# actcwlf/GSVC

Hardware: NVIDIA B200
Metric: train_iters_per_s (higher is better)
Workload: dtype f32

## Files before the change

gsvc_b200/csrc/common.cuh:

```cuda
#pragma once

#include <cuda_runtime.h>
#include <stdint.h>
#include <stddef.h>

#include "../../include/gsvc_rast.h"

namespace gsvc {

constexpr int TILE = GSVC_RAST_TILE;
constexpr int TILE_PIX = TILE * TILE;
constexpr float ALPHA_MIN = 1.0f / 255.0f;
constexpr float ALPHA_MAX = 0.99f;
constexpr float T_STOP = 0.0001f;
constexpr float LOWPASS = 0.3f;

constexpr int MAX_VIEWS = GSVC_RAST_MAX_VIEWS;
struct ViewTable {
    const float* V[MAX_VIEWS];
    long long vs_r[MAX_VIEWS], vs_c[MAX_VIEWS];
    float campos[MAX_VIEWS][3];
    int out_image[MAX_VIEWS];
    int flip_x[MAX_VIEWS];
    float weight[MAX_VIEWS];
};

struct DevSettings {
    int W, H, gx, gy;
    float x_min, y_min, scale, threshold, scale_modifier;
    const float* bg;
    int sh_degree, sh_M;
    int n_views, accumulate;
    ViewTable vt;
};

struct GeomView {
    float4* feat0;
    float4* feat1;
    float4* feat2;
    float4* feat3;
    ushort4* rect;
    uint8_t* clamped;
};

struct ImageHeader {
    unsigned long long num_rendered;
    unsigned int overflow;
    unsigned int n_heavy;
    unsigned int pad[28];
};
struct ImageView {
    ImageHeader* hdr;
    unsigned int* tile_count;
    unsigned long long* scan_partials;
    unsigned int* tile_offset;
    unsigned int* tile_cursor;
    uint2* ranges;
    unsigned int* heavy_tiles;
    float* final_T;
    unsigned int* n_contrib;
};

struct BinView {
    unsigned long long* inst;
    unsigned int* point_list;
    unsigned int* depth_keys;
};

__host__ __device__ inline size_t align_up(size_t x, size_t a) { return (x + a - 1) / a * a; }

template <typename T>
__host__ __device__ inline T* carve(char*& p, size_t count)
{
    T* r = reinterpret_cast<T*>(p);
    p += align_up(count * sizeof(T), 256);
    return r;
}

inline GeomView geom_view(void* buf, int P, int sh_M)
{
    char* p = static_cast<char*>(buf);
    GeomView g;
    g.feat0 = carve<float4>(p, P);
    g.feat1 = carve<float4>(p, P);
    g.feat2 = carve<float4>(p, P);
    g.feat3 = carve<float4>(p, P);
    g.rect = carve<ushort4>(p, P);
    g.clamped = sh_M > 0 ? carve<uint8_t>(p, (size_t)P * 3) : nullptr;
    return g;
}
inline size_t geom_bytes(int P, int sh_M)
{
    char* p = nullptr;
    carve<float4>(p, P); carve<float4>(p, P); carve<float4>(p, P); carve<float4>(p, P); carve<ushort4>(p, P);
    if (sh_M > 0) carve<uint8_t>(p, (size_t)P * 3);
    return (size_t)p + 256;
}
inline ImageView image_view(void* buf, int W, int H, int n_views = 1)
{
    char* p = static_cast<char*>(buf);
    size_t T = (size_t)((W + TILE - 1) / TILE) * ((H + TILE - 1) / TILE) * n_views;
    size_t N = (size_t)W * H * n_views;
    ImageView v;
    v.hdr = carve<ImageHeader>(p, 1);
    v.tile_count = carve<unsigned int>(p, T);
    v.scan_partials = carve<unsigned long long>(p, T / 1024 + 2);
    v.tile_offset = carve<unsigned int>(p, T);
    v.tile_cursor = carve<unsigned int>(p, T);
    v.ranges = carve<uint2>(p, T);
    v.heavy_tiles = carve<unsigned int>(p, T);
    v.final_T = carve<float>(p, N);
    v.n_contrib = carve<unsigned int>(p, N);
    return v;
}
inline size_t image_bytes(int W, int H, int n_views = 1)
{
    char* p = nullptr;
    size_t T = (size_t)((W + TILE - 1) / TILE) * ((H + TILE - 1) / TILE) * n_views;
    size_t N = (size_t)W * H * n_views;
    carve<ImageHeader>(p, 1); carve<unsigned int>(p, T); carve<unsigned long long>(p, T / 1024 + 2);
    carve<unsigned int>(p, T); carve<unsigned int>(p, T); carve<uint2>(p, T); carve<unsigned int>(p, T); carve<float>(p, N);
    carve<unsigned int>(p, N);
    return (size_t)p + 256;
}
inline BinView bin_view(void* buf, long long cap)
{
    char* p = static_cast<char*>(buf);
    BinView b;
    b.inst = carve<unsigned long long>(p, (size_t)cap);
    b.point_list = carve<unsigned int>(p, (size_t)cap);
    b.depth_keys = carve<unsigned int>(p, (size_t)cap);
    return b;
}
inline size_t bin_bytes(long long cap)
{
    char* p = nullptr;
    carve<unsigned long long>(p, (size_t)cap); carve<unsigned int>(p, (size_t)cap); carve<unsigned int>(p, (size_t)cap);
    return (size_t)p + 256;
}

inline size_t bwd_scratch_bytes(int P) { return align_up((size_t)P * 48, 256) + 256; }

__host__ __device__ inline unsigned int ordered_u32(float z)
{
#ifdef __CUDA_ARCH__
    unsigned int u = __float_as_uint(z);
#else
    unsigned int u; memcpy(&u, &z, 4);
#endif
    return (u & 0x80000000u) ? ~u : (u | 0x80000000u);
}

__device__ __forceinline__ float4 ld_row4(const float* __restrict__ base, size_t row)
{
    if ((reinterpret_cast<uintptr_t>(base) & 15u) == 0u) return __ldg(reinterpret_cast<const float4*>(base) + row);
    const float* p = base + 4 * row;
    return make_float4(__ldg(p), __ldg(p + 1), __ldg(p + 2), __ldg(p + 3));
}
__device__ __forceinline__ void st_row4(float* __restrict__ base, size_t row, float4 v)
{
    if ((reinterpret_cast<uintptr_t>(base) & 15u) == 0u) { reinterpret_cast<float4*>(base)[row] = v; return; }
    float* p = base + 4 * row;
    p[0] = v.x; p[1] = v.y; p[2] = v.z; p[3] = v.w;
}

#define GSVC_MUL(a, b) __fmul_rn((a), (b))
#define GSVC_ADD(a, b) __fadd_rn((a), (b))
#define GSVC_SUB(a, b) __fsub_rn((a), (b))

__device__ __forceinline__ void quat_to_rot(const float4 q, float R[9])
{
    const float r = q.x, x = q.y, y = q.z, z = q.w;
    R[0] = GSVC_SUB(1.f, GSVC_MUL(2.f, GSVC_ADD(GSVC_MUL(y, y), GSVC_MUL(z, z))));
    R[1] = GSVC_MUL(2.f, GSVC_SUB(GSVC_MUL(x, y), GSVC_MUL(r, z)));
    R[2] = GSVC_MUL(2.f, GSVC_ADD(GSVC_MUL(x, z), GSVC_MUL(r, y)));
    R[3] = GSVC_MUL(2.f, GSVC_ADD(GSVC_MUL(x, y), GSVC_MUL(r, z)));
    R[4] = GSVC_SUB(1.f, GSVC_MUL(2.f, GSVC_ADD(GSVC_MUL(x, x), GSVC_MUL(z, z))));
    R[5] = GSVC_MUL(2.f, GSVC_SUB(GSVC_MUL(y, z), GSVC_MUL(r, x)));
    R[6] = GSVC_MUL(2.f, GSVC_SUB(GSVC_MUL(x, z), GSVC_MUL(r, y)));
    R[7] = GSVC_MUL(2.f, GSVC_ADD(GSVC_MUL(y, z), GSVC_MUL(r, x)));
    R[8] = GSVC_SUB(1.f, GSVC_MUL(2.f, GSVC_ADD(GSVC_MUL(x, x), GSVC_MUL(y, y))));
}

__device__ __forceinline__ float dot3_rn(float a0, float b0, float a1, float b1, float a2, float b2)
{
    return GSVC_ADD(GSVC_ADD(GSVC_MUL(a0, b0), GSVC_MUL(a1, b1)), GSVC_MUL(a2, b2));
}

__device__ __forceinline__ void cov3d_from_scale_rot(const float* s3, float mod, const float4 q, float cov[6])
{
    float R[9], M[9];
    quat_to_rot(q, R);
    const float sx = GSVC_MUL(mod, s3[0]), sy = GSVC_MUL(mod, s3[1]), sz = GSVC_MUL(mod, s3[2]);
#pragma unroll
    for (int i = 0; i < 3; i++) {
        M[3 * i + 0] = GSVC_MUL(R[3 * i + 0], sx);
        M[3 * i + 1] = GSVC_MUL(R[3 * i + 1], sy);
        M[3 * i + 2] = GSVC_MUL(R[3 * i + 2], sz);
    }
    cov[0] = dot3_rn(M[0], M[0], M[1], M[1], M[2], M[2]);
    cov[1] = dot3_rn(M[0], M[3], M[1], M[4], M[2], M[5]);
    cov[2] = dot3_rn(M[0], M[6], M[1], M[7], M[2], M[8]);
    cov[3] = dot3_rn(M[3], M[3], M[4], M[4], M[5], M[5]);
    cov[4] = dot3_rn(M[3], M[6], M[4], M[7], M[5], M[8]);
    cov[5] = dot3_rn(M[6], M[6], M[7], M[7], M[8], M[8]);
}

__device__ __forceinline__ void cov2d_ortho(const float cov[6], const float w0[3], const float w1[3], float scale,
                                            float& a, float& b, float& c)
{
    const float u00 = dot3_rn(cov[0], w0[0], cov[1], w0[1], cov[2], w0[2]);
    const float u01 = dot3_rn(cov[1], w0[0], cov[3], w0[1], cov[4], w0[2]);
    const float u02 = dot3_rn(cov[2], w0[0], cov[4], w0[1], cov[5], w0[2]);
    const float u10 = dot3_rn(cov[0], w1[0], cov[1], w1[1], cov[2], w1[2]);
    const float u11 = dot3_rn(cov[1], w1[0], cov[3], w1[1], cov[4], w1[2]);
    const float u12 = dot3_rn(cov[2], w1[0], cov[4], w1[1], cov[5], w1[2]);
    const float s2 = GSVC_MUL(scale, scale);
    a = GSVC_ADD(GSVC_MUL(s2, dot3_rn(w0[0], u00, w0[1], u01, w0[2], u02)), LOWPASS);
    b = GSVC_MUL(s2, dot3_rn(w0[0], u10, w0[1], u11, w0[2], u12));
    c = GSVC_ADD(GSVC_MUL(s2, dot3_rn(w1[0], u10, w1[1], u11, w1[2], u12)), LOWPASS);
}

__device__ __forceinline__ void pdl_prologue()
{
#if defined(__CUDA_ARCH__)
    asm volatile("griddepcontrol.launch_dependents;");
    asm volatile("griddepcontrol.wait;" ::: "memory");
#endif
}

template <typename... KArgs, typename... Args>
inline cudaError_t launch_pdl(void (*kernel)(KArgs...), dim3 grid, dim3 block, cudaStream_t st, Args... args)
{
    cudaLaunchConfig_t cfg = {};
    cfg.gridDim = grid;
    cfg.blockDim = block;
    cfg.dynamicSmemBytes = 0;
    cfg.stream = st;
    cudaLaunchAttribute attr[1];
    attr[0].id = cudaLaunchAttributeProgrammaticStreamSerialization;
    attr[0].val.programmaticStreamSerializationAllowed = 1;
    cfg.attrs = attr;
    cfg.numAttrs = 1;
    return cudaLaunchKernelEx(&cfg, kernel, KArgs(args)...);
}

struct WarpTiles {
    int incl, excl, total;
    int rx, ry, rw;
};

__device__ __forceinline__ WarpTiles warp_tiles_begin(int area, int rx, int ry, int rw)
{
    const int lane = threadIdx.x & 31;
    int v = area;
#pragma unroll
    for (int d = 1; d < 32; d <<= 1) {
        const int o = __shfl_up_sync(0xffffffffu, v, d);
        if (lane >= d) v += o;
    }
    WarpTiles w;
    w.incl = v; w.excl = v - area; w.total = __shfl_sync(0xffffffffu, v, 31);
    w.rx = rx; w.ry = ry; w.rw = rw;
    return w;
}

__device__ __forceinline__ int warp_tiles_get(const WarpTiles& w, int idx, int gx, int& owner)
{
    int o = 0;
#pragma unroll
    for (int step = 16; step >= 1; step >>= 1) {
        const int v = __shfl_sync(0xffffffffu, w.incl, o + step - 1);
        if (v <= idx) o += step;
    }
    o = min(o, 31);
    const int local = idx - __shfl_sync(0xffffffffu, w.excl, o);
    const int rw = __shfl_sync(0xffffffffu, w.rw, o);
    const int rx = __shfl_sync(0xffffffffu, w.rx, o), ry = __shfl_sync(0xffffffffu, w.ry, o);
    owner = o;
    if (idx >= w.total) return -1;
    int row = __float2int_rz(__fdividef(__int2float_rz(local), __int2float_rz(rw)));
    int rem = local - row * rw;
    if (rem < 0) { row--; rem += rw; }
    else if (rem >= rw) { row++; rem -= rw; }
    return (ry + row) * gx + rx + rem;
}

struct PreInputs {
    int P;
    const float* means3D;
    const float* shs;
    const float* colors_precomp;
    const float* opacities;
    const float* scales;
    const float* rotations;
    const float* cov3D_precomp;
    int range_lo, range_hi;
};

cudaError_t launch_visible_filter(const DevSettings& s, const PreInputs& in, int32_t* radii, cudaStream_t st);
inline size_t compact_scratch_bytes(int P)
{
    const size_t n = ((size_t)(P < 1 ? 1 : P) + 255) / 256;
    return 256 + 2 * align_up(n * 4, 256) + align_up(n * 32, 256) + 256;
}
cudaError_t launch_visible_filter_compact(const DevSettings& s, const PreInputs& in, int32_t* radii, int32_t* indices,
                                          void* scratch, unsigned long long* host_slot, unsigned int ticket,
                                          cudaStream_t st);
cudaError_t launch_preprocess(const DevSettings& s, const PreInputs& in, int32_t* radii, GeomView g, ImageView im,
                              float4* acc_to_zero, cudaStream_t st);
cudaError_t launch_tile_scan(const DevSettings& s, ImageView im, unsigned long long* host_slot, unsigned int ticket,
                             cudaStream_t st);
cudaError_t launch_scatter(const DevSettings& s, int P, GeomView g, ImageView im, BinView b, long long cap,
                           bool count_overflow_events, cudaStream_t st);
cudaError_t launch_sort_tiles(const DevSettings& s, ImageView im, BinView b, long long cap, cudaStream_t st);
cudaError_t launch_render_forward(const DevSettings& s, GeomView g, ImageView im, BinView b, long long cap,
                                  float* out_color, cudaStream_t st);
cudaError_t launch_render_backward(const DevSettings& s, int P, GeomView g, ImageView im, BinView b, long long cap,
                                   const float* dL_dout, float4* acc, bool acc_is_zero, cudaStream_t st);
struct BwdOutputs {
    float* dL_dmeans3D; float* dL_dmeans2D; float* dL_dcolors; float* dL_dopacities;
    float* dL_dscales; float* dL_drotations; float* dL_dcov3D; float* dL_dshs;
    float* packed;
};
struct ExchangeArgs {
    float4* mc;
    float4* const* bufs;
    unsigned int* const* pads;
    unsigned int* state;
    int rank, world;
    int n_ex;
    int chunk_ctas, n_chunks;
    int n_compute;
    long long chunk_f4, total_f4;
};
cudaError_t launch_preprocess_backward(const DevSettings& s, const PreInputs& in, const int32_t* radii, GeomView g,
                                       const float4* acc, BwdOutputs out, ExchangeArgs ex, cudaStream_t st);
cudaError_t launch_export_keys(const DevSettings& s, ImageView im, BinView b, long long R,
                               unsigned long long* sorted_keys, unsigned int* point_list, unsigned int* ranges,
                               cudaStream_t st);
cudaError_t launch_export_geom(int P, GeomView g, float* depth, float* xy, float* conic_opacity, float* rgb,
                               int32_t* rect, cudaStream_t st);

cudaError_t read_overflow_events(unsigned int* host_value, bool reset, cudaStream_t st);
cudaError_t launch_densify_stats(int n_views, int P, const float* dm2d, const int32_t* radii, float* stats,
                                 long long stride, bool accumulate, cudaStream_t st);

cudaError_t launch_switch_allreduce(float* multicast, void* const* buffers, unsigned int* const* pads, unsigned int* state,
                                    int rank, int world, long long numel, int n_ctas, cudaStream_t st);
void count_launch(int n = 1);

}
```

gsvc_b200/csrc/render.cu:

```cuda
#include "common.cuh"

namespace gsvc {

constexpr int BLEND_THREADS = 128;
constexpr int BATCH = 256;
constexpr unsigned FULL = 0xffffffffu;

__device__ __forceinline__ float ex2_approx(float x)
{
    float y;
    asm("ex2.approx.ftz.f32 %0, %1;" : "=f"(y) : "f"(x));
    return y;
}
__device__ __forceinline__ float rcp_approx(float x)
{
    float y;
    asm("rcp.approx.ftz.f32 %0, %1;" : "=f"(y) : "f"(x));
    return y;
}

struct f2 { unsigned long long v; };
__device__ __forceinline__ f2 mk2(float lo, float hi)
{
    f2 r;
    asm("mov.b64 %0, {%1, %2};" : "=l"(r.v) : "f"(lo), "f"(hi));
    return r;
}
__device__ __forceinline__ f2 bc2(float s) { return mk2(s, s); }
__device__ __forceinline__ float lo(f2 a)
{
    float x;
    [[maybe_unused]] float y;
    asm("mov.b64 {%0, %1}, %2;" : "=f"(x), "=f"(y) : "l"(a.v));
    return x;
}
__device__ __forceinline__ float hi(f2 a)
{
    [[maybe_unused]] float x;
    float y;
    asm("mov.b64 {%0, %1}, %2;" : "=f"(x), "=f"(y) : "l"(a.v));
    return y;
}
__device__ __forceinline__ f2 fma2(f2 a, f2 b, f2 c)
{
    f2 r;
    asm("fma.rn.f32x2 %0, %1, %2, %3;" : "=l"(r.v) : "l"(a.v), "l"(b.v), "l"(c.v));
    return r;
}
__device__ __forceinline__ void fma2_acc(f2& c, f2 a, f2 b)
{
    asm("fma.rn.f32x2 %0, %1, %2, %0;" : "+l"(c.v) : "l"(a.v), "l"(b.v));
}
__device__ __forceinline__ f2 mul2(f2 a, f2 b)
{
    f2 r;
    asm("mul.rn.f32x2 %0, %1, %2;" : "=l"(r.v) : "l"(a.v), "l"(b.v));
    return r;
}
__device__ __forceinline__ f2 add2(f2 a, f2 b)
{
    f2 r;
    asm("add.rn.f32x2 %0, %1, %2;" : "=l"(r.v) : "l"(a.v), "l"(b.v));
    return r;
}
__device__ __forceinline__ f2 sub2(f2 a, f2 b)
{
    f2 r;
    asm("sub.rn.f32x2 %0, %1, %2;" : "=l"(r.v) : "l"(a.v), "l"(b.v));
    return r;
}
__device__ __forceinline__ f2 neg2(f2 a) { return mk2(-lo(a), -hi(a)); }

__device__ __forceinline__ f2 neg_falloff_log2(float rho_hi, const float4 f1, float dx, f2 dy2, f2& u2, f2& v2)
{
    const f2 t2 = fma2(bc2(f1.y), dy2, fma2(bc2(rho_hi), dy2, bc2(dx)));
    u2 = mul2(bc2(f1.x), t2);
    v2 = mul2(bc2(f1.z), dy2);
    return fma2(u2, u2, mul2(v2, v2));
}
__device__ __forceinline__ f2 neg_falloff_log2(float rho_hi, const float4 f1, float dx, f2 dy2)
{
    f2 u2, v2;
    return neg_falloff_log2(rho_hi, f1, dx, dy2, u2, v2);
}

struct BlockGeom {
    int px, py;
    float xmin, xmax, ymin, ymax;
};

__device__ __forceinline__ BlockGeom block_geom(int tile, int gx, int tid)
{
    const int tx = tile % gx, ty = tile / gx;
    const int warp = tid >> 5, lane = tid & 31;
    const int bx0 = tx * TILE + (warp & 1) * 8, by0 = ty * TILE + (warp >> 1) * 8;
    BlockGeom b;
    b.px = bx0 + (lane & 7);
    b.py = by0 + (lane >> 3);
    b.xmin = (float)bx0; b.xmax = (float)(bx0 + 7);
    b.ymin = (float)by0; b.ymax = (float)(by0 + 7);
    return b;
}

constexpr float CULL_MARGIN = 1e-3f;

__device__ __forceinline__ void stage(float4* s_feat, int slot, const GeomView& geo, unsigned int id)
{
    const float4 f0 = __ldg(geo.feat0 + id);
    const float4 f1 = __ldg(geo.feat3 + id);
    float4 f2 = __ldg(geo.feat2 + id);
    f2.w = __uint_as_float(id);
    s_feat[3 * slot] = f0;
    s_feat[3 * slot + 1] = f1;
    s_feat[3 * slot + 2] = f2;
}

__device__ __forceinline__ bool block_hit(const BlockGeom& b, const float4* e)
{
    const float4 f0 = e[0];
    const float4 f1 = e[1];
    const float thr = -__log2f(255.0f * f1.w) - CULL_MARGIN;
    const float ex = fminf(fmaxf(f0.x, b.xmin), b.xmax), ey = fminf(fmaxf(f0.y, b.ymin), b.ymax);
    const float dxe = ex - f0.x, dye = ey - f0.y;
    const float dy1 = fminf(fmaxf(fmaf(-f0.w, dxe, f0.y), b.ymin), b.ymax) - f0.y;
    const float dx2 = fminf(fmaxf(fmaf(-f0.z, dye, f0.x), b.xmin), b.xmax) - f0.x;
    const float u1 = f1.x * fmaf(f0.z, dy1, dxe), v1 = f1.z * dy1;
    const float u2 = f1.x * fmaf(f0.z, dye, dx2), v2 = f1.z * dye;
    const float nq1 = fmaf(u1, u1, v1 * v1), nq2 = fmaf(u2, u2, v2 * v2);
    return -fminf(nq1, nq2) >= thr;
}

__global__ void __launch_bounds__(BLEND_THREADS)
render_forward_kernel(DevSettings s, GeomView geo, ImageView im, BinView bin, unsigned long long cap,
                      float* __restrict__ out_color)
{
    __shared__ float4 s_feat[3 * BATCH];

    pdl_prologue();
    const int Tv = s.gx * s.gy;
    const int view = (int)blockIdx.x / Tv;
    const int tile = (int)blockIdx.x - view * Tv;
    const int tid = threadIdx.x, lane = tid & 31;
    const BlockGeom bg = block_geom(tile, s.gx, tid);
    const bool inA = bg.px < s.W && bg.py < s.H, inB = bg.px < s.W && bg.py + 4 < s.H;
    const float pxf = (float)bg.px, pyf = (float)bg.py;

    const uint2 rg = im.ranges[blockIdx.x];
    if ((unsigned long long)rg.y > cap) return;
    const int n = (int)(rg.y - rg.x);

    float TA = 1.f, A0 = 0.f, A1 = 0.f, A2 = 0.f;
    float TB = 1.f, B0 = 0.f, B1 = 0.f, B2 = 0.f;
    const f2 npy2 = mk2(-pyf, -(pyf + 4.f));
    unsigned int lastA = 0, lastB = 0;
    constexpr float DONE = 2.f;
    float minA = inA ? ALPHA_MIN : DONE, minB = inB ? ALPHA_MIN : DONE;

    for (int base = 0; base < n; base += BATCH) {
        if (__syncthreads_count(minA > 1.f && minB > 1.f) == BLEND_THREADS) break;
#pragma unroll
        for (int r = 0; r < BATCH / BLEND_THREADS; r++) {
            const int slot = tid + r * BLEND_THREADS;
            if (base + slot < n) stage(s_feat, slot, geo, bin.point_list[rg.x + base + slot]);
        }
        __syncthreads();
        const int cnt = min(BATCH, n - base);
        for (int c = 0; c < cnt; c += 32) {
            if (__ballot_sync(FULL, !(minA > 1.f && minB > 1.f)) == 0u) break;
            bool hit = false;
            if (c + lane < cnt) hit = block_hit(bg, s_feat + 3 * (c + lane));
            unsigned int m = __ballot_sync(FULL, hit);
            const float4* chunk = s_feat + 3 * c;
            const unsigned int pos1 = (unsigned int)(base + c + 1);
            while (m) {
                const int k = __ffs(m) - 1;
                m &= m - 1;
                const float4* e = chunk + 3 * k;
                const float4 f0 = e[0];
                const float4 f1 = e[1];
                const float4 f2v = e[2];
                const f2 nq2 = neg_falloff_log2(f0.z, f1, f0.x - pxf, add2(bc2(f0.y), npy2));
                const f2 a2 = mul2(bc2(f1.w), mk2(ex2_approx(-lo(nq2)), ex2_approx(-hi(nq2))));
                const float aA = fminf(ALPHA_MAX, lo(a2)), aB = fminf(ALPHA_MAX, hi(a2));
                const bool okA = !(aA < minA);
                const bool okB = !(aB < minB);
                const unsigned int pos = pos1 + (unsigned int)k;
                const f2 ac = mk2(aA, aB), T2 = mk2(TA, TB);
                const f2 tT2 = mul2(T2, sub2(bc2(1.f), ac));
                const f2 w2 = mul2(ac, T2);
                const float tTA = lo(tT2), tTB = hi(tT2);
                if (okA && tTA < T_STOP) minA = DONE;
                if (okB && tTB < T_STOP) minB = DONE;
                const bool addA = okA && !(tTA < T_STOP), addB = okB && !(tTB < T_STOP);
                const f2 wz = mk2(addA ? lo(w2) : 0.f, addB ? hi(w2) : 0.f);
                { const f2 c = fma2(bc2(f2v.x), wz, mk2(A0, B0)); A0 = lo(c); B0 = hi(c); }
                { const f2 c = fma2(bc2(f2v.y), wz, mk2(A1, B1)); A1 = lo(c); B1 = hi(c); }
                { const f2 c = fma2(bc2(f2v.z), wz, mk2(A2, B2)); A2 = lo(c); B2 = hi(c); }
                if (addA) { TA = tTA; lastA = pos; }
                if (addB) { TB = tTB; lastB = pos; }
            }
        }
    }
    const size_t N = (size_t)s.W * s.H;
    const float bg0 = __ldg(s.bg + 0), bg1 = __ldg(s.bg + 1), bg2 = __ldg(s.bg + 2);
    float* const fT = im.final_T + (size_t)view * N;
    unsigned int* const nc = im.n_contrib + (size_t)view * N;
    float* const out = out_color + (size_t)s.vt.out_image[view] * 3 * N;
    const float wgt = s.vt.weight[view];
    const int ox = s.vt.flip_x[view] ? s.W - 1 - bg.px : bg.px;
    if (inA) {
        const size_t pix = (size_t)bg.py * s.W + bg.px, opix = (size_t)bg.py * s.W + ox;
        const float c0 = wgt * (A0 + TA * bg0), c1 = wgt * (A1 + TA * bg1), c2 = wgt * (A2 + TA * bg2);
        if (s.accumulate) {
            atomicAdd(out + opix, c0); atomicAdd(out + N + opix, c1); atomicAdd(out + 2 * N + opix, c2);
        } else {
            out[opix] = c0; out[N + opix] = c1; out[2 * N + opix] = c2;
        }
        fT[pix] = TA;
        nc[pix] = lastA;
    }
    if (inB) {
        const size_t pix = (size_t)(bg.py + 4) * s.W + bg.px, opix = (size_t)(bg.py + 4) * s.W + ox;
        const float c0 = wgt * (B0 + TB * bg0), c1 = wgt * (B1 + TB * bg1), c2 = wgt * (B2 + TB * bg2);
        if (s.accumulate) {
            atomicAdd(out + opix, c0); atomicAdd(out + N + opix, c1); atomicAdd(out + 2 * N + opix, c2);
        } else {
            out[opix] = c0; out[N + opix] = c1; out[2 * N + opix] = c2;
        }
        fT[pix] = TB;
        nc[pix] = lastB;
    }
}

cudaError_t launch_render_forward(const DevSettings& s, GeomView g, ImageView im, BinView b, long long cap,
                                  float* out_color, cudaStream_t st)
{
    const int T = s.gx * s.gy * s.n_views;
    if (T <= 0) return cudaSuccess;
    count_launch();
    return launch_pdl(render_forward_kernel, dim3(T), dim3(BLEND_THREADS), st, s, g, im, b, (unsigned long long)cap,
                      out_color);
}

constexpr int BWD_THREADS = 64;
constexpr int BWD_STAGE = BATCH / BWD_THREADS;

struct QuadBwd {
    f2 T01, T23, Sg01, Sg23;
    f2 g0_01, g0_23, g1_01, g1_23, g2_01, g2_23;
    unsigned int last0, last1, last2, last3;
};

__device__ __forceinline__ float half_reduce8(float v[8], int lane)
{
    bool hi = lane & 8;
#pragma unroll
    for (int i = 0; i < 4; i++) {
        const float send = hi ? v[i] : v[i + 4];
        const float keep = hi ? v[i + 4] : v[i];
        v[i] = keep + __shfl_xor_sync(FULL, send, 8);
    }
    hi = lane & 4;
#pragma unroll
    for (int i = 0; i < 2; i++) {
        const float send = hi ? v[i] : v[i + 2];
        const float keep = hi ? v[i + 2] : v[i];
        v[i] = keep + __shfl_xor_sync(FULL, send, 4);
    }
    hi = lane & 2;
    {
        const float send = hi ? v[0] : v[1];
        const float keep = hi ? v[1] : v[0];
        v[0] = keep + __shfl_xor_sync(FULL, send, 2);
    }
    v[0] += __shfl_xor_sync(FULL, v[0], 1);
    return v[0];
}

__device__ __forceinline__ float half_sum(float v)
{
#pragma unroll
    for (int d = 8; d >= 1; d >>= 1) v += __shfl_xor_sync(FULL, v, d);
    return v;
}

__global__ void __launch_bounds__(BWD_THREADS, 12)
render_backward_kernel(DevSettings s, GeomView geo, ImageView im, BinView bin, unsigned long long cap,
                       const float* __restrict__ dL_dout, float* __restrict__ acc )
{
    __shared__ float4 s_feat[3 * BATCH];
    __shared__ unsigned char s_list[2][2][BATCH];
    __shared__ unsigned int s_max[2];

    pdl_prologue();
    const int Tv = s.gx * s.gy;
    const int view = (int)blockIdx.x / Tv;
    const int tile = (int)blockIdx.x - view * Tv;
    const int tid = threadIdx.x, lane = tid & 31, warp = tid >> 5, half = lane >> 4, l16 = lane & 15;
    const unsigned int lt_mask = (1u << lane) - 1u;
    const int tx = tile % s.gx, ty = tile / s.gx;
    const int by0 = ty * TILE + warp * 8;
    const int bx0 = tx * TILE + half * 8;
    const int px = bx0 + (l16 & 7), py0 = by0 + (l16 >> 3);
    BlockGeom gA, gB;
    gA.px = gB.px = 0; gA.py = gB.py = 0;
    gA.xmin = (float)(tx * TILE); gA.xmax = gA.xmin + 7.f; gB.xmin = gA.xmin + 8.f; gB.xmax = gB.xmin + 7.f;
    gA.ymin = gB.ymin = (float)by0; gA.ymax = gB.ymax = (float)(by0 + 7);
    const size_t N = (size_t)s.W * s.H;
    const float wgt = s.vt.weight[view];
    const float* const dL = dL_dout + (size_t)s.vt.out_image[view] * 3 * N;
    const float* const fT = im.final_T + (size_t)view * N;
    const unsigned int* const nc = im.n_contrib + (size_t)view * N;
    const int ox = s.vt.flip_x[view] ? s.W - 1 - px : px;

    const uint2 rg = im.ranges[blockIdx.x];
    const int n = (int)(rg.y - rg.x);
    if (n <= 0) return;
    if ((unsigned long long)rg.y > cap || im.hdr->overflow != 0u) return;

    unsigned int spec_id[BWD_STAGE];
#pragma unroll
    for (int r = 0; r < BWD_STAGE; r++) {
        const int kp = n - 1 - (tid + r * BWD_THREADS);
        spec_id[r] = kp >= 0 ? __ldg(bin.point_list + rg.x + kp) : 0u;
    }

    const float bg0 = __ldg(s.bg), bg1 = __ldg(s.bg + 1), bg2 = __ldg(s.bg + 2);
    QuadBwd S;
    {
        float T[4], Sg[4], g0[4], g1[4], g2[4];
        unsigned int last[4];
#pragma unroll
        for (int i = 0; i < 4; i++) {
            const int py = py0 + 2 * i;
            T[i] = 0.f; Sg[i] = 0.f; g0[i] = g1[i] = g2[i] = 0.f; last[i] = 0u;
            if (px < s.W && py < s.H) {
                const size_t pix = (size_t)py * s.W + px, opix = (size_t)py * s.W + ox;
                T[i] = fT[pix]; last[i] = nc[pix];
                g0[i] = wgt * dL[opix]; g1[i] = wgt * dL[N + opix]; g2[i] = wgt * dL[2 * N + opix];
                Sg[i] = T[i] * (bg0 * g0[i] + bg1 * g1[i] + bg2 * g2[i]);
            }
        }
        S.T01 = mk2(T[0], T[1]); S.T23 = mk2(T[2], T[3]); S.Sg01 = mk2(Sg[0], Sg[1]); S.Sg23 = mk2(Sg[2], Sg[3]);
        S.g0_01 = mk2(g0[0], g0[1]); S.g0_23 = mk2(g0[2], g0[3]); S.g1_01 = mk2(g1[0], g1[1]); S.g1_23 = mk2(g1[2], g1[3]);
        S.g2_01 = mk2(g2[0], g2[1]); S.g2_23 = mk2(g2[2], g2[3]);
        S.last0 = last[0]; S.last1 = last[1]; S.last2 = last[2]; S.last3 = last[3];
    }
    const float pxf = (float)px, pyf = (float)py0;
    const f2 npy01 = mk2(-pyf, -(pyf + 2.f)), npy23 = mk2(-(pyf + 4.f), -(pyf + 6.f));

    const unsigned int lmax = max(max(S.last0, S.last1), max(S.last2, S.last3));
    const unsigned int hmaxA = __reduce_max_sync(FULL, half == 0 ? lmax : 0u);
    const unsigned int hmaxB = __reduce_max_sync(FULL, half == 1 ? lmax : 0u);
    if (lane == 0) s_max[warp] = max(hmaxA, hmaxB);
    __syncthreads();
    const int m_len = min((int)max(s_max[0], s_max[1]), n);

    const int red_lane = ((l16 & 1) == 0 || l16 == 1) ? 1 : 0;
    const int red_off = l16 == 1 ? 8 : (((l16 >> 3) & 1) * 4 + ((l16 >> 2) & 1) * 2 + ((l16 >> 1) & 1));

    for (int base = 0; base < m_len; base += BATCH) {
        __syncthreads();
#pragma unroll
        for (int r = 0; r < BWD_STAGE; r++) {
            const int slot = tid + r * BWD_THREADS;
            const int kpos = m_len - 1 - (base + slot);
            if (kpos >= 0) {
                const unsigned int id = (base == 0 && m_len == n) ? spec_id[r] : bin.point_list[rg.x + kpos];
                stage(s_feat, slot, geo, id);
            }
        }
        __syncthreads();
        const int cnt = min(BATCH, m_len - base);
        const int posb = m_len - 1 - base;
        int nA = 0, nB = 0;
        for (int c = 0; c < cnt; c += 32) {
            const int pos = posb - c - lane;
            bool hitA = false, hitB = false;
            if (c + lane < cnt) {
                const float4* e = s_feat + 3 * (c + lane);
                if ((unsigned int)pos < hmaxA) hitA = block_hit(gA, e);
                if ((unsigned int)pos < hmaxB) hitB = block_hit(gB, e);
            }
            const unsigned int mA = __ballot_sync(FULL, hitA), mB = __ballot_sync(FULL, hitB);
            if (hitA) s_list[warp][0][nA + __popc(mA & lt_mask)] = (unsigned char)(c + lane);
            if (hitB) s_list[warp][1][nB + __popc(mB & lt_mask)] = (unsigned char)(c + lane);
            nA += __popc(mA); nB += __popc(mB);
        }
        __syncwarp();
        const int nh = half ? nB : nA;
        const int iters = max(nA, nB);
        const unsigned char* const list = s_list[warp][half];
        for (int it = 0; it < iters; it++) {
            const bool valid = it < nh;
            const int k = valid ? (int)list[it] : 0;
            const float4* e = s_feat + 3 * k;
            const float4 f0 = e[0];
            const float4 f1 = e[1];
            const float4 f2v = e[2];
            const float dx = f0.x - pxf;
            const f2 dy01 = add2(bc2(f0.y), npy01), dy23 = add2(bc2(f0.y), npy23);
            f2 u01, v01, u23, v23;
            const f2 nq01 = neg_falloff_log2(f0.z, f1, dx, dy01, u01, v01);
            const f2 nq23 = neg_falloff_log2(f0.z, f1, dx, dy23, u23, v23);
            const f2 a01 = mul2(bc2(f1.w), mk2(ex2_approx(-lo(nq01)), ex2_approx(-hi(nq01))));
            const f2 a23 = mul2(bc2(f1.w), mk2(ex2_approx(-lo(nq23)), ex2_approx(-hi(nq23))));
            const unsigned int pos = (unsigned int)(posb - k);
            const bool u0 = valid && (pos < S.last0) && !(lo(a01) < ALPHA_MIN);
            const bool u1 = valid && (pos < S.last1) && !(hi(a01) < ALPHA_MIN);
            const bool u2 = valid && (pos < S.last2) && !(lo(a23) < ALPHA_MIN);
            const bool u3 = valid && (pos < S.last3) && !(hi(a23) < ALPHA_MIN);
            const f2 am01 = mk2(u0 ? lo(a01) : 0.f, u1 ? hi(a01) : 0.f);
            const f2 am23 = mk2(u2 ? lo(a23) : 0.f, u3 ? hi(a23) : 0.f);
            const f2 ae01 = mk2(fminf(ALPHA_MAX, lo(am01)), fminf(ALPHA_MAX, hi(am01)));
            const f2 ae23 = mk2(fminf(ALPHA_MAX, lo(am23)), fminf(ALPHA_MAX, hi(am23)));
            const f2 om01 = sub2(bc2(1.f), ae01), om23 = sub2(bc2(1.f), ae23);
            const f2 ra01 = mk2(rcp_approx(lo(om01)), rcp_approx(hi(om01)));
            const f2 ra23 = mk2(rcp_approx(lo(om23)), rcp_approx(hi(om23)));
            S.T01 = mul2(S.T01, ra01); S.T23 = mul2(S.T23, ra23);
            const f2 cg01 = fma2(bc2(f2v.x), S.g0_01, fma2(bc2(f2v.y), S.g1_01, mul2(bc2(f2v.z), S.g2_01)));
            const f2 cg23 = fma2(bc2(f2v.x), S.g0_23, fma2(bc2(f2v.y), S.g1_23, mul2(bc2(f2v.z), S.g2_23)));
            const f2 dla01 = fma2(S.T01, cg01, neg2(mul2(ra01, S.Sg01)));
            const f2 dla23 = fma2(S.T23, cg23, neg2(mul2(ra23, S.Sg23)));
            const f2 dch01 = mul2(ae01, S.T01), dch23 = mul2(ae23, S.T23);
            S.Sg01 = fma2(dch01, cg01, S.Sg01); S.Sg23 = fma2(dch23, cg23, S.Sg23);
            const f2 w01 = mul2(am01, dla01), w23 = mul2(am23, dla23);
            const f2 wu01 = mul2(w01, u01), wu23 = mul2(w23, u23), wv01 = mul2(w01, v01), wv23 = mul2(w23, v23);
            const f2 s_wu = add2(wu01, wu23), s_wv = add2(wv01, wv23);
            const f2 s_wuu = fma2(wu01, u01, mul2(wu23, u23)), s_wuv = fma2(wu01, v01, mul2(wu23, v23));
            const f2 s_wvv = fma2(wv01, v01, mul2(wv23, v23)), s_w = add2(w01, w23);
            const f2 s_r = fma2(dch01, S.g0_01, mul2(dch23, S.g0_23)), s_g = fma2(dch01, S.g1_01, mul2(dch23, S.g1_23));
            const f2 s_b = fma2(dch01, S.g2_01, mul2(dch23, S.g2_23));
            float v[8];
            v[0] = lo(s_wu) + hi(s_wu);
            v[1] = lo(s_wv) + hi(s_wv);
            v[2] = lo(s_wuu) + hi(s_wuu);
            v[3] = lo(s_wuv) + hi(s_wuv);
            v[4] = lo(s_wvv) + hi(s_wvv);
            v[5] = lo(s_w) + hi(s_w);
            v[6] = lo(s_r) + hi(s_r);
            v[7] = lo(s_g) + hi(s_g);
            float d_b = lo(s_b) + hi(s_b);
            const float sum8 = half_reduce8(v, lane);
            d_b = half_sum(d_b);
            if (red_lane && valid) atomicAdd(acc + (size_t)__float_as_uint(f2v.w) * 12 + red_off, l16 == 1 ? d_b : sum8);
        }
    }
}


cudaError_t launch_render_backward(const DevSettings& s, int P, GeomView g, ImageView im, BinView b, long long cap,
                                   const float* dL_dout, float4* acc, bool acc_is_zero, cudaStream_t st)
{
    if (!acc_is_zero) {
        cudaError_t e = cudaMemsetAsync(acc, 0, (size_t)P * s.n_views * 48, st);
        if (e != cudaSuccess) return e;
    }
    const int T = s.gx * s.gy * s.n_views;
    if (T <= 0 || P <= 0) return cudaSuccess;
    count_launch();
    return launch_pdl(render_backward_kernel, dim3(T), dim3(BWD_THREADS), st, s, g, im, b, (unsigned long long)cap,
                      dL_dout, reinterpret_cast<float*>(acc));
}

}
```

Measured before the change: 4693.

## Cache forward per-subblock hit masks and reuse them in backward culling

The forward blend kernel now writes each warp's ballot hit mask per 32-entry chunk into a new per-instance uint4 buffer. The backward kernel reads these masks instead of recomputing block_hit against two 8x8 subblock geometries, and skips staging features for entries no subblock touches. This removes geometry tests and some shared-memory staging loads in backward, at the cost of extra global writes in forward, extra global reads in backward, and a larger bin buffer. It assumes forward and backward use the same subblock partitioning and that the forward loop covers every chunk; chunks skipped by forward's early exit leave masks unwritten.

Result: slower. 4643 (median of 6 runs) (-1.1%).

```diff
diff --git a/gsvc_b200/csrc/common.cuh b/gsvc_b200/csrc/common.cuh
--- a/gsvc_b200/csrc/common.cuh
+++ b/gsvc_b200/csrc/common.cuh
@@ -65,6 +65,7 @@
     unsigned long long* inst;
     unsigned int* point_list;
     unsigned int* depth_keys;
+    uint4* hit_masks;
 };
 
 __host__ __device__ inline size_t align_up(size_t x, size_t a) { return (x + a - 1) / a * a; }
@@ -130,12 +131,14 @@
     b.inst = carve<unsigned long long>(p, (size_t)cap);
     b.point_list = carve<unsigned int>(p, (size_t)cap);
     b.depth_keys = carve<unsigned int>(p, (size_t)cap);
+    b.hit_masks = carve<uint4>(p, (size_t)cap);
     return b;
 }
 inline size_t bin_bytes(long long cap)
 {
     char* p = nullptr;
     carve<unsigned long long>(p, (size_t)cap); carve<unsigned int>(p, (size_t)cap); carve<unsigned int>(p, (size_t)cap);
+    carve<uint4>(p, (size_t)cap);
     return (size_t)p + 256;
 }
 
diff --git a/gsvc_b200/csrc/render.cu b/gsvc_b200/csrc/render.cu
--- a/gsvc_b200/csrc/render.cu
+++ b/gsvc_b200/csrc/render.cu
@@ -170,6 +170,7 @@
             bool hit = false;
             if (c + lane < cnt) hit = block_hit(bg, s_feat + 3 * (c + lane));
             unsigned int m = __ballot_sync(FULL, hit);
+            if (lane == 0) reinterpret_cast<unsigned int*>(bin.hit_masks + rg.x + base + c)[tid >> 5] = m;
             const float4* chunk = s_feat + 3 * c;
             const unsigned int pos1 = (unsigned int)(base + c + 1);
             while (m) {
@@ -284,12 +285,20 @@
     return v;
 }
 
+__device__ __forceinline__ unsigned int hit_flags(const BinView& bin, unsigned int start, int k)
+{
+    const uint4 m = __ldg(bin.hit_masks + start + (k & ~31));
+    const int s = k & 31;
+    return ((m.x >> s) & 1u) | (((m.y >> s) & 1u) << 1) | (((m.z >> s) & 1u) << 2) | (((m.w >> s) & 1u) << 3);
+}
+
 __global__ void __launch_bounds__(BWD_THREADS, 12)
 render_backward_kernel(DevSettings s, GeomView geo, ImageView im, BinView bin, unsigned long long cap,
                        const float* __restrict__ dL_dout, float* __restrict__ acc )
 {
     __shared__ float4 s_feat[3 * BATCH];
     __shared__ unsigned char s_list[2][2][BATCH];
+    __shared__ unsigned char s_flag[BATCH];
     __shared__ unsigned int s_max[2];
 
     pdl_prologue();
@@ -302,10 +311,6 @@
     const int by0 = ty * TILE + warp * 8;
     const int bx0 = tx * TILE + half * 8;
     const int px = bx0 + (l16 & 7), py0 = by0 + (l16 >> 3);
-    BlockGeom gA, gB;
-    gA.px = gB.px = 0; gA.py = gB.py = 0;
-    gA.xmin = (float)(tx * TILE); gA.xmax = gA.xmin + 7.f; gB.xmin = gA.xmin + 8.f; gB.xmax = gB.xmin + 7.f;
-    gA.ymin = gB.ymin = (float)by0; gA.ymax = gB.ymax = (float)(by0 + 7);
     const size_t N = (size_t)s.W * s.H;
     const float wgt = s.vt.weight[view];
     const float* const dL = dL_dout + (size_t)s.vt.out_image[view] * 3 * N;
@@ -319,10 +324,12 @@
     if ((unsigned long long)rg.y > cap || im.hdr->overflow != 0u) return;
 
     unsigned int spec_id[BWD_STAGE];
+    unsigned int spec_f = 0u;
 #pragma unroll
     for (int r = 0; r < BWD_STAGE; r++) {
         const int kp = n - 1 - (tid + r * BWD_THREADS);
         spec_id[r] = kp >= 0 ? __ldg(bin.point_list + rg.x + kp) : 0u;
+        if (kp >= 0) spec_f |= hit_flags(bin, rg.x, kp) << (8 * r);
     }
 
     const float bg0 = __ldg(s.bg), bg1 = __ldg(s.bg + 1), bg2 = __ldg(s.bg + 2);
@@ -365,23 +372,23 @@
         for (int r = 0; r < BWD_STAGE; r++) {
             const int slot = tid + r * BWD_THREADS;
             const int kpos = m_len - 1 - (base + slot);
-            if (kpos >= 0) {
-                const unsigned int id = (base == 0 && m_len == n) ? spec_id[r] : bin.point_list[rg.x + kpos];
+            const bool spec = base == 0 && m_len == n;
+            unsigned int f = 0u;
+            if (kpos >= 0) f = spec ? (spec_f >> (8 * r)) & 0xffu : hit_flags(bin, rg.x, kpos);
+            if (kpos >= 0 && (f != 0u || slot == 0)) {
+                const unsigned int id = spec ? spec_id[r] : bin.point_list[rg.x + kpos];
                 stage(s_feat, slot, geo, id);
             }
+            s_flag[slot] = (unsigned char)f;
         }
         __syncthreads();
         const int cnt = min(BATCH, m_len - base);
         const int posb = m_len - 1 - base;
         int nA = 0, nB = 0;
         for (int c = 0; c < cnt; c += 32) {
-            const int pos = posb - c - lane;
-            bool hitA = false, hitB = false;
-            if (c + lane < cnt) {
-                const float4* e = s_feat + 3 * (c + lane);
-                if ((unsigned int)pos < hmaxA) hitA = block_hit(gA, e);
-                if ((unsigned int)pos < hmaxB) hitB = block_hit(gB, e);
-            }
+            const unsigned int pos = (unsigned int)(posb - c - lane), f = s_flag[c + lane];
+            const bool hitA = ((f >> (2 * warp)) & 1u) && pos < hmaxA;
+            const bool hitB = ((f >> (2 * warp + 1)) & 1u) && pos < hmaxB;
             const unsigned int mA = __ballot_sync(FULL, hitA), mB = __ballot_sync(FULL, hitB);
             if (hitA) s_list[warp][0][nA + __popc(mA & lt_mask)] = (unsigned char)(c + lane);
             if (hitB) s_list[warp][1][nB + __popc(mB & lt_mask)] = (unsigned char)(c + lane);
```
